# jaeyoungjo99/ELiMaLoc

Hardware: AMD Instinct MI355X
Metric: ICP registrations/sec, 128k-pt scan vs 10M-pt map; pose err vs CPU ref (higher is better)
Workload: dtype f64

## Files before the change

### elimaloc_amd/_lib.py

```python
import ctypes as C
import os

_HERE = os.path.dirname(os.path.abspath(__file__))
LIB_PATH = os.environ.get("ELM_LIB") or os.path.join(_HERE, "libelimaloc_hip.so")

ELM_OK = 0
P2P, GICP, VGICP, AVGICP = 0, 1, 2, 3
MAX_ITER_TRACE = 64
PACKED_SUMS = 32
COMM_ID_BYTES = 128


class ElmError(RuntimeError):
    pass


class RegConfig(C.Structure):
    _fields_ = [
        ("i_max_thread", C.c_int32),
        ("icp_method", C.c_int32),
        ("voxel_search_method", C.c_int32),
        ("use_radar_cov", C.c_int32),
        ("max_iteration", C.c_int32),
        ("b_debug_print", C.c_int32),
# ... 124 lines not shown


class FreeSpaceStatsC(C.Structure):
    _fields_ = [("n_counted", C.c_uint32), ("n_pierced", C.c_uint32), ("n_end_occupied", C.c_uint32), ("n_supported", C.c_uint32),
                ("n_samples", C.c_uint64), ("n_hit_samples", C.c_uint64)]


class RayCastConfigC(C.Structure):
    _fields_ = [("sub", C.c_int32), ("max_steps", C.c_int32), ("min_range_m", C.c_double), ("max_range_m", C.c_double),
                ("cmp_min_range_m", C.c_double), ("cmp_max_range_m", C.c_double), ("tol_m", C.c_double), ("tol_frac", C.c_double),
                ("origin", C.c_double * 3)]


class RayCastStatsC(C.Structure):
    _fields_ = [("n_cast", C.c_uint32), ("n_hit", C.c_uint32), ("n_miss", C.c_uint32), ("n_truncated", C.c_uint32),
                ("n_compared", C.c_uint32), ("n_match", C.c_uint32), ("n_through", C.c_uint32), ("n_front", C.c_uint32),
                ("n_steps", C.c_uint64)]


ALLREDUCE_FN = C.CFUNCTYPE(C.c_int, C.c_void_p, C.c_size_t, C.c_void_p, C.c_void_p)

EXPORTS = [
    "elm_reg_config_default", "elm_ctx_create", "elm_ctx_create_multi", "elm_ctx_group_info", "elm_register_shard", "elm_ctx_destroy", "elm_last_error", "elm_strerror",
    "elm_ctx_synchronize", "elm_ctx_stream", "elm_ctx_set_profiling", "elm_ctx_set_work_counters", "elm_ctx_get_profile", "elm_map_build", "elm_map_destroy", "elm_map_cal_voxel_cov_all",
    "elm_map_cal_point_cov_all", "elm_map_build_neighbourhoods", "elm_map_get_info", "elm_map_empty", "elm_map_download_points",
    "elm_map_download_voxels", "elm_map_find_ground_height", "elm_map_get_correspondences", "elm_align_clouds_local", "elm_scan_upload", "elm_scan_destroy",
    "elm_scan_size", "elm_scan_download", "elm_register", "elm_format_register_log", "elm_register_batch", "elm_register_stream", "elm_register_stream_host", "elm_host_alloc", "elm_host_free", "elm_ctx_measure_h2d", "elm_register_batch_enqueue",
    "elm_register_batch_finish", "elm_deskew", "elm_deskew_downsample", "elm_deskew_prepare", "elm_comm_get_unique_id", "elm_comm_init",
    "elm_comm_destroy", "elm_comm_info", "elm_comm_set_hook", "elm_filter_points_by_distance", "elm_voxel_downsample",
    "elm_get_interpolated_pose", "elm_shape_odom_covariance", "elm_cal_frame_point_cov",
    "elm_ekf_config_default", "elm_ekf_create", "elm_ekf_destroy", "elm_ekf_predict_imu", "elm_ekf_predict", "elm_ekf_update_can", "elm_gps_project", "elm_ekf_update_navsatfix",
    "elm_ekf_update_pose", "elm_ekf_update_pcm_odom", "elm_ekf_get_state", "elm_ekf_publish",
    "elm_ini_load", "elm_ini_destroy", "elm_ini_get_string", "elm_ini_get_int", "elm_ini_get_bool", "elm_ini_get_double",
    "elm_ini_get_array", "elm_pcm_node_config_default", "elm_load_pcm_config", "elm_load_ekf_config", "elm_pcd_load_xyz",
    "elm_free", "elm_scan_from_cloud", "elm_pcm_callback_point_cloud",
    "elm_reloc_config_default", "elm_reloc_make_hypotheses", "elm_map_score_poses", "elm_relocalize",
    "elm_reloc_global_config_default", "elm_map_ground_heights", "elm_reloc_global_hypotheses", "elm_relocalize_global",
    "elm_freespace_config_default", "elm_map_fine_cells", "elm_map_check_free_space",
    "elm_raycast_config_default", "elm_map_raycast",
]


class PcmNodeConfig(C.Structure):
    _fields_ = [("lidar_type", C.c_char * 32), ("lidar_scan_time_end", C.c_int32), ("pcm_voxel_max_point", C.c_int32),
                ("run_deskew", C.c_int32), ("input_index_sampling", C.c_int32), ("lidar_time_delay", C.c_double),
                ("pcm_voxel_size", C.c_double), ("input_max_dist", C.c_double), ("input_voxel_ds_m", C.c_double),
                ("tf_ego_to_lidar", C.c_double * 16)]
# ... 49 lines not shown
                       "(hipcc --offload-arch=gfx950). There is no CPU fallback.")
    L = C.CDLL(LIB_PATH, mode=C.RTLD_GLOBAL)
    vp, dp, fp, ip = C.c_void_p, C.POINTER(C.c_double), C.POINTER(C.c_float), C.POINTER(C.c_int)
    L.elm_reg_config_default.argtypes = [C.POINTER(RegConfig)]
    L.elm_reg_config_default.restype = None
    L.elm_ctx_create.argtypes = [C.c_int, C.POINTER(vp)]
    L.elm_ctx_destroy.argtypes = [vp]
    L.elm_ctx_create_multi.argtypes = [C.POINTER(C.c_int), C.c_int, C.POINTER(vp)]
    L.elm_ctx_group_info.argtypes = [vp, C.POINTER(C.c_int), C.POINTER(C.c_int), C.POINTER(C.c_int), C.c_int]
    L.elm_register_shard.argtypes = [vp, vp, fp, C.c_size_t, C.c_size_t, dp, C.POINTER(RegConfig), C.POINTER(RegResult), C.POINTER(IterTrace), C.c_int]
    L.elm_ctx_destroy.restype = None
    L.elm_last_error.argtypes = [vp]
    L.elm_last_error.restype = C.c_char_p
    L.elm_strerror.argtypes = [C.c_int]
    L.elm_strerror.restype = C.c_char_p
    L.elm_ctx_synchronize.argtypes = [vp]
    L.elm_ctx_stream.argtypes = [vp]
    L.elm_ctx_stream.restype = vp
    L.elm_format_register_log.argtypes = [C.POINTER(RegConfig), C.POINTER(RegResult), C.c_size_t, C.POINTER(IterTrace), C.POINTER(C.c_double),
                                          C.c_double, C.c_char_p, C.c_size_t]
    L.elm_format_register_log.restype = C.c_size_t
    L.elm_ctx_set_profiling.argtypes = [vp, C.c_int]
    L.elm_ctx_set_work_counters.argtypes = [vp, C.c_int]
    L.elm_ctx_get_profile.argtypes = [vp, C.POINTER(Profile), C.c_int]
    L.elm_map_build.argtypes = [vp, fp, C.c_size_t, C.c_double, C.c_int, C.POINTER(vp)]
    L.elm_map_destroy.argtypes = [vp]
    L.elm_map_destroy.restype = None
    L.elm_map_cal_voxel_cov_all.argtypes = [vp]
    L.elm_map_cal_point_cov_all.argtypes = [vp, C.c_double]
    L.elm_map_build_neighbourhoods.argtypes = [vp]
    L.elm_map_get_info.argtypes = [vp, C.POINTER(MapInfo)]
    L.elm_map_empty.argtypes = [vp]
    L.elm_map_download_points.argtypes = [vp, dp, dp, dp, C.c_size_t]
    L.elm_map_download_voxels.argtypes = [vp, C.POINTER(C.c_int32), C.POINTER(C.c_int32), dp, dp, C.c_size_t]
    L.elm_map_find_ground_height.argtypes = [vp, C.c_double, C.c_double, dp, ip]
    L.elm_cal_frame_point_cov.argtypes = [dp, C.c_size_t, C.c_double, C.c_double, C.c_double, dp]
    L.elm_align_clouds_local.argtypes = [vp, C.c_int, dp, dp, dp, dp, C.c_size_t, dp, C.c_double, C.POINTER(RegConfig), dp, dp, dp]
    L.elm_map_get_correspondences.argtypes = [vp, vp, C.c_int, dp, C.c_size_t, C.c_double, C.POINTER(C.c_uint32), C.POINTER(C.c_int32), C.c_size_t, C.POINTER(C.c_size_t)]
    L.elm_scan_upload.argtypes = [vp, fp, C.c_size_t, C.c_size_t, C.POINTER(vp)]
    L.elm_scan_destroy.argtypes = [vp]
    L.elm_scan_destroy.restype = None
    L.elm_scan_size.argtypes = [vp]
    L.elm_scan_size.restype = C.c_size_t
    L.elm_scan_download.argtypes = [vp, fp, C.c_size_t]
    L.elm_deskew_downsample.argtypes = [vp, fp, fp, C.c_size_t, C.POINTER(DeskewTables), C.c_double, C.POINTER(vp), ip]
    L.elm_register.argtypes = [vp, vp, fp, C.c_size_t, dp, C.POINTER(RegConfig), dp, ip, dp, dp,
# ... 96 lines not shown
```

### elimaloc_amd/csrc/elm_api.cpp

```cpp
#include <dlfcn.h>
#include <hip/hip_runtime.h>
#include <math.h>
#include <stdio.h>
#include <stdlib.h>
#include <string.h>
#include <unistd.h>

#include <algorithm>
#include <array>
#include <chrono>
#include <map>
#include <mutex>
#include <new>
#include <set>
#include <string>
#include <thread>
#include <vector>

#include "elm_hostapi.hpp"
#include "elm_internal.hpp"
#include "elm_la.hpp"

using namespace elm;

// ... 48 lines not shown
    g_rccl.comm_init_rank = (nccl_comm_init_rank_t)dlsym(h, "ncclCommInitRank");
    g_rccl.all_reduce = (nccl_all_reduce_t)dlsym(h, "ncclAllReduce");
    g_rccl.comm_destroy = (nccl_comm_destroy_t)dlsym(h, "ncclCommDestroy");
    g_rccl.get_error_string = (nccl_get_error_string_t)dlsym(h, "ncclGetErrorString");
    g_rccl.comm_count = (nccl_comm_query_t)dlsym(h, "ncclCommCount");
    g_rccl.comm_user_rank = (nccl_comm_query_t)dlsym(h, "ncclCommUserRank");
    if (!g_rccl.get_unique_id || !g_rccl.comm_init_rank || !g_rccl.all_reduce || !g_rccl.comm_destroy) {
        if (err) *err = "librccl lacks ncclGetUniqueId/ncclCommInitRank/ncclAllReduce/ncclCommDestroy";
        return false;
    }
    g_rccl.handle = h;
    return true;
}

struct elm_ctx {
    int device = 0;
    uint64_t id = 0;
    hipStream_t stream = nullptr;
    hipStream_t copy_stream = nullptr, order_stream = nullptr, poll_stream = nullptr;
    hipEvent_t ev_iter[4] = {nullptr, nullptr, nullptr, nullptr};
    std::vector<hipEvent_t> ev_groups;
    uint16_t* d_hilbert = nullptr;
    DevBuf d_order_jobs, d_order_tmp, d_arena, d_raw, d_flagged, d_asym;
    DevBuf d_q0, d_q1, d_q2, d_q3, d_q4, d_q5;
    DevBuf d_reloc[16];
    bool work_counters = false;
    void* h_jobs = nullptr;
    size_t h_jobs_cap = 0;
    std::string last_error;
    DevBuf d_scans, d_state, d_partials, d_sums, d_T0, d_trace, d_stage_pts, d_active, d_queue, d_ds;
    int stream_hint_count = 0, stream_hint_slots = 0, stream_hint_iters = 0;
    int* h_active = nullptr;
    int iter_hint = 0;
    int iter_ring[8] = {0, 0, 0, 0, 0, 0, 0, 0};
    unsigned iter_ring_pos = 0;
    const void* iter_key_map = nullptr;
    int iter_key_method = -1, iter_key_batch = 0;
    void* h_state = nullptr;
    size_t h_state_cap = 0;
    void* h_trace = nullptr;
    size_t h_trace_cap = 0;
    void* h_stage = nullptr;
    size_t h_stage_cap = 0;
    std::vector<uint32_t> h_key, h_ord, h_tmp;
    std::vector<struct elm_scan*> scan_free;
    std::vector<std::pair<void*, size_t>> scan_pool;
// ... 161 lines not shown
}

extern "C" void elm_ctx_destroy(elm_ctx* ctx) {
    if (!ctx) return;
    if (ctx->group && !elm_multi::in_worker()) {
        elm_group* g = ctx->group;
        elm_multi::destroy(g);
    }
    {
        std::lock_guard<std::mutex> lk(g_live_mu);
        if (!g_live_ctx.erase(ctx)) return;
    }
    (void)hipSetDevice(ctx->device);
    if (ctx->stream) (void)hipStreamSynchronize(ctx->stream);
    if (ctx->comm && g_rccl.comm_destroy) g_rccl.comm_destroy(ctx->comm);
    for (hipStream_t st : {ctx->copy_stream, ctx->order_stream, ctx->poll_stream})
        if (st) { (void)hipStreamSynchronize(st); (void)hipStreamDestroy(st); }
    for (hipEvent_t e : {ctx->ev_iter[0], ctx->ev_iter[1], ctx->ev_iter[2], ctx->ev_iter[3]})
        if (e) (void)hipEventDestroy(e);
    for (hipEvent_t e : ctx->ev_groups) (void)hipEventDestroy(e);
    if (ctx->d_hilbert) (void)hipFree(ctx->d_hilbert);
    if (ctx->h_jobs) (void)hipHostFree(ctx->h_jobs);
    DevBuf* bufs[] = {&ctx->d_scans, &ctx->d_state, &ctx->d_partials, &ctx->d_sums, &ctx->d_T0, &ctx->d_trace, &ctx->d_stage_pts, &ctx->d_active, &ctx->d_queue, &ctx->d_ds,
                      &ctx->d_order_jobs, &ctx->d_order_tmp, &ctx->d_arena, &ctx->d_raw, &ctx->d_flagged, &ctx->d_asym, &ctx->d_q0, &ctx->d_q1, &ctx->d_q2, &ctx->d_q3, &ctx->d_q4, &ctx->d_q5};
    if (ctx->h_active) (void)hipHostFree(ctx->h_active);
    for (DevBuf* b : bufs)
        if (b->p) (void)hipFree(b->p);
    for (DevBuf& b : ctx->d_reloc)
        if (b.p) (void)hipFree(b.p);
    for (auto& b : ctx->scan_pool) (void)hipFree(b.first);
    for (elm_scan* f : ctx->scan_free) delete f;
    if (ctx->h_state) (void)hipHostFree(ctx->h_state);
    if (ctx->h_trace) (void)hipHostFree(ctx->h_trace);
    if (ctx->h_stage) (void)hipHostFree(ctx->h_stage);
    if (ctx->h_desc) (void)hipHostFree(ctx->h_desc);
    for (hipEvent_t e : ctx->events) (void)hipEventDestroy(e);
    if (ctx->stream) (void)hipStreamDestroy(ctx->stream);
    delete ctx;
}

extern "C" const char* elm_last_error(const elm_ctx* ctx) { return ctx ? ctx->last_error.c_str() : ""; }
extern "C" void* elm_ctx_stream(elm_ctx* ctx) { return ctx ? (void*)ctx->stream : nullptr; }
extern "C" int elm_ctx_set_work_counters(elm_ctx* ctx, int enable) {
    if (!ctx) return ELM_ERR_INVALID;
    if (ctx->in_flight) return ELM_ERR_INVALID;
    if (group_call(ctx)) return elm_multi::set_work_counters(ctx, enable);
    ctx->work_counters = enable != 0;
    return ELM_OK;
}

extern "C" int elm_ctx_set_profiling(elm_ctx* ctx, int enable) {
    if (!ctx) return ELM_ERR_INVALID;
    ctx->profiling = enable != 0;
    return ELM_OK;
}
extern "C" int elm_ctx_get_profile(elm_ctx* ctx, elm_profile* out, int reset) {
    if (!ctx || !out) return ELM_ERR_INVALID;
    *out = ctx->prof;
    if (reset) ctx->prof = elm_profile{};
    return ELM_OK;
}
static int prof_mark(elm_ctx* ctx) {
    if (!ctx->profiling) return ELM_OK;
    if (ctx->events_used == (int)ctx->events.size()) {
        hipEvent_t e;
        HIPCHK(ctx, hipEventCreateWithFlags(&e, hipEventDisableSystemFence));
        ctx->events.push_back(e);
    }
    HIPCHK(ctx, hipEventRecord(ctx->events[ctx->events_used++], ctx->stream));
    return ELM_OK;
// ... 1563 lines not shown
    RegParams rp;
    memset(&rp, 0, sizeof(rp));
    rp.th = cfg->max_search_dist;
    rp.th2 = cfg->max_search_dist * cfg->max_search_dist;
    rp.lm_lambda = cfg->lm_lambda;
    rp.term_thr = cfg->icp_termination_threshold_m;
    rp.min_overlap = cfg->min_overlap_ratio;
    rp.max_fitness = cfg->max_fitness_score;
    rp.method = cfg->icp_method;
    rp.max_iter = cfg->max_iteration;
    rp.uniform_blocks = uniform_blocks;
    rp.radar = pc.radar ? (cfg->use_radar_cov != 0 ? 1 : 2) : 0;
    rp.stats = ctx->work_counters ? 1 : 0;
    rp.radar_var[0] = cfg->range_variance_m;
    rp.radar_var[1] = cfg->azimuth_variance_deg;
    rp.radar_var[2] = cfg->elevation_variance_deg;
    if (pc.asym) {
        int rc;
        if ((rc = dev_reserve(ctx, ctx->d_asym, (size_t)std::max<uint32_t>(blocks, 1) * kAsymRecord * sizeof(double))) != ELM_OK) return rc;
        rp.asym = (double*)ctx->d_asym.p;
        rp.asym_sums = (double*)ctx->d_sums.p + (size_t)n_scans * kSums;
    }
    rp.rank_check = ((ctx->comm || ctx->hook) && !rp.radar && !rp.stats) ? 1 : 0;
    ctx->rp = rp;
    return ELM_OK;
}

static bool reg_args_ok(const elm_ctx* ctx, const elm_map* map, const elm_reg_config* cfg) {
    return map->ctx == ctx && cfg->icp_method >= ELM_P2P && cfg->icp_method <= ELM_AVGICP && !ctx->in_flight;
}

struct StateTail {
    int32_t active;
    int32_t rank_mismatch;
    int32_t _pad0[2];
    uint32_t ds_kept;
    int32_t ds_overflow;
    int32_t _pad1[10];
};
static_assert(sizeof(StateTail) == 64 && offsetof(StateTail, rank_mismatch) == 4 && offsetof(StateTail, ds_kept) == 16 &&
              offsetof(StateTail, ds_overflow) == 20, "the state tail's layout");
static StateTail* state_tail(void* states, int n_scans) { return (StateTail*)((char*)states + (size_t)n_scans * sizeof(ScanState)); }

static size_t trace_bytes(int count) { return (size_t)count * ELM_MAX_ITER_TRACE * sizeof(elm_iter_trace); }
static int reserve_trace(elm_ctx* ctx, int count, elm_iter_trace** d_trace) {
    const size_t tb = trace_bytes(count);
// ... 1169 lines not shown
```

### elimaloc_amd/csrc/elm_internal.hpp

```cpp
#pragma once
#include <hip/hip_runtime.h>
#include <stdint.h>

#include "../../include/elimaloc_hip.h"

namespace elm {

struct __attribute__((aligned(32))) HashSlot {
    int32_t kx, ky, kz;
    int32_t vid;
    uint32_t start;
    uint32_t cnt;
    uint32_t pad0, pad1;
};

struct __attribute__((packed, aligned(4))) Pt3 {
    float x, y, z;
};

struct __attribute__((aligned(16))) GridBlk {
    float x[4], y[4], z[4];
};

struct __attribute__((aligned(64))) VoxRec {
// ... 123 lines not shown
};

struct RegParams {
    double th;
    double th2;
    double lm_lambda;
    double term_thr;
    double min_overlap;
    double max_fitness;
    int32_t method;
    int32_t max_iter;
    uint32_t uniform_blocks;
    int32_t radar;
    int32_t _reserved0;
    int32_t stats;
    uint32_t* flagged;
    int32_t rank_check;
    int32_t _pad_rc;
    double* asym;
    double* asym_sums;
    double radar_var[3];
    const double* query;
    int32_t* q_out;
};
constexpr int kAsymRecord = 16;
constexpr int kRadarRecord = 64;

constexpr int kTileShift = 3, kTile = 1 << kTileShift;
constexpr int kBlock = 256;
constexpr int kInitPack = 8;
struct InitPack {
    ScanDesc d[kInitPack];
    double T0[kInitPack][16];
};
constexpr int kSums = ELM_PACKED_SUMS;

void launch_init_state(hipStream_t s, ScanState* st, const double* T0, int batch, int map_empty, int* active);
void launch_init_pack(hipStream_t s, ScanDesc* scans, ScanState* st, const InitPack& pack, int batch, int map_empty, int* active, const unsigned* n_dev);
void launch_stream_refill(hipStream_t s, ScanDesc* scans, ScanState* st, int slots, const QueueItem* queue, const double* qT0,
                          ScanState* out_state, StreamCtrl* ctrl, int first, int save = 1);
void launch_accumulate_radar(hipStream_t s, const DevMap& m, const ScanDesc* scans, int batch, int total_blocks, ScanState* st, double* partials,
                             const RegParams& rp);
void launch_accumulate_direct(hipStream_t s, const DevMap& m, const ScanDesc* scans, int batch, int total_blocks,
                              ScanState* st, double* partials, const RegParams& rp);
void launch_solve(hipStream_t s, const ScanDesc* scans, int batch, ScanState* st, const double* partials,
                  double* sums, const RegParams& rp, elm_iter_trace* trace, int mode, int* active, const StreamArgs* refill = nullptr);
// ... 129 lines not shown
```

### elimaloc_amd/csrc/elm_k_grid.hip

```cpp
#include <float.h>
#include <algorithm>
#include <hip/hip_runtime.h>

#include "elm_internal.hpp"
#include "elm_la.hpp"
#include "elm_dev_grid.hpp"

namespace elm {

template <int METHOD, int COMPACT, int TILED, int STATS, int WIDE>
__global__ __launch_bounds__(kBlock, (METHOD == ELM_P2P ? (STATS ? 7 : kGridWaves) : kGicpWaves)) void k_accumulate_grid(
       const DevMap m, const ScanDesc* __restrict__ scans, int batch,
                                                                            unsigned total_blocks, const ScanState* __restrict__ st,
                                                                            double* __restrict__ partials, const RegParams rp) {
    constexpr int kStats = (STATS == 1) ? 1 : 0;
    constexpr bool QUERY = STATS == 2;
    constexpr int NV = (METHOD == ELM_P2P) ? (kStats ? kP2PVals : kP2PVals - 3) : kSums;
    __shared__ double s_buf[kRedPass * kBlock];
    __shared__ double s_red[kSums];
    __shared__ int s_res[kBlock];
    __shared__ int s_tst[kStats ? kBlock : 1];
    __shared__ float s_pz[METHOD == ELM_P2P ? kBlock : 1];
    __shared__ unsigned s_st[kStats ? kBlock : 1];
    __shared__ unsigned s_cnt[kBlock / 64];
    const unsigned L = xcd_remap(blockIdx.x, total_blocks);
    const int s = find_scan(scans, batch, L, rp);
    const ScanState& S = st[s];
    if (S.done) return;
    const ScanDesc sd = scans[s];
    if (L >= sd.blk_end) return;
    const unsigned i = (L - sd.blk_begin) * kBlock + threadIdx.x;
    const bool valid = i < sd.n;
    double v[(METHOD == ELM_P2P) ? NV : 1];
#pragma unroll
    for (int k = 0; k < ((METHOD == ELM_P2P) ? NV : 1); ++k) v[k] = 0.0;
    PairSum P;
    if (METHOD != ELM_P2P) pair_sum_zero(P);
    int bj = -1;
    int n_tested = 0;
    float hr2 = __builtin_inff();
    bool hard = false;
    const double h = 0.5 * m.voxel_size;
    const GridBlk* __restrict__ lp = m.grid_blk;
    constexpr unsigned kBlkStep = WIDE ? (unsigned)(sizeof(GridBlk) / 16) : (unsigned)sizeof(GridBlk);
    auto stash_w = [&](double a, double b, double c, double d) {
        double* p = s_buf + threadIdx.x;
        p[4 * kBlock] = a; p[5 * kBlock] = b; p[6 * kBlock] = c; p[7 * kBlock] = d;
    };
    auto load_g = [&](double& gx, double& gy, double& gz, float& pxf, float& pyf) {
        const double* p = s_buf + threadIdx.x;
        gx = p[4 * kBlock]; gy = p[5 * kBlock]; gz = p[6 * kBlock];
        const double w = p[7 * kBlock];
        pxf = __int_as_float(__double2loint(w)); pyf = __int_as_float(__double2hiint(w));
    };
    auto transform = [&](const float4 pf, double& px, double& py, double& pz, double& gx, double& gy, double& gz) {
        px = pf.x; py = pf.y; pz = pf.z;
        gx = ((S.T[0] * px + S.T[4] * py) + S.T[8] * pz) + S.T[12];
        gy = ((S.T[1] * px + S.T[5] * py) + S.T[9] * pz) + S.T[13];
        gz = ((S.T[2] * px + S.T[6] * py) + S.T[10] * pz) + S.T[14];
    };
    if (valid) {
        double px, py, pz, gx, gy, gz;
        float4 pf = make_float4(0.f, 0.f, 0.f, 0.f);
        if (QUERY) {
            gx = rp.query[3 * (size_t)i]; gy = rp.query[3 * (size_t)i + 1]; gz = rp.query[3 * (size_t)i + 2];
            px = py = pz = 0.0;
        } else {
            const Pt3 p3 = sd.pts[i];
            pf = make_float4(p3.x, p3.y, p3.z, 0.f);
            transform(pf, px, py, pz, gx, gy, gz);
        }
        const GridAxis ax = grid_axis(gx, m), ay = grid_axis(gy, m), az = grid_axis(gz, m);
        unsigned stat = 0;
        if (kStats && !TILED) {
            const int ux = ax.f - m.vx0, uy = ay.f - m.vy0, uz = az.f - m.vz0;
            const bool in_box = (unsigned)ux < (unsigned)m.vnx && (unsigned)uy < (unsigned)m.vny && (unsigned)uz < (unsigned)m.vnz;
            const unsigned sidx = in_box ? ((unsigned)ux * (unsigned)m.vny + (unsigned)uy) * (unsigned)m.vnz + (unsigned)uz : 0u;
            stat = m.vox_stat[sidx];
            stat = in_box ? stat : 0u;
        }
        float rho_u = 3e38f;
        int bx0, bx1, by0, by1, bz0, bz1;
        int ox, oy, oz;
        float dxo, dyo, dzo;
        grid_lean(ax, bx0, bx1, rho_u, ox, dxo);
        grid_lean(ay, by0, by1, rho_u, oy, dyo);
        grid_lean(az, bz0, bz1, rho_u, oz, dzo);
        (void)oz; (void)dzo;
        const int rx0 = bx0 - m.gx0, rx1 = bx1 - m.gx0, ry0 = by0 - m.gy0, ry1 = by1 - m.gy0, rz0 = bz0 - m.gz0, rz1 = bz1 - m.gz0;
        const bool inside = rx0 >= 0 && rx1 < m.gnx && rx0 <= rx1 && ry0 >= 0 && ry1 < m.gny && ry0 <= ry1 && rz0 >= 0 && rz1 < m.gnz && rz0 <= rz1;
        unsigned sb[4];
        int cb[5];
        cb[0] = 0;
        const float ex_ = fmaxf(dxo * (float)h - 1e-6f, 0.f), ey_ = fmaxf(dyo * (float)h - 1e-6f, 0.f);
        const float Bx = fminf(ex_ * ex_, 1e36f), By = fminf(ey_ * ey_, 1e36f);
        const bool xfirst = Bx <= By, has_x = rx1 != rx0, has_y = ry1 != ry0;
        unsigned s0[4], s1[4], s2[4];
        bool ok[4];
        ok[0] = inside;
        ok[1] = inside && (xfirst ? has_x : has_y);
        ok[2] = inside && (xfirst ? has_y : has_x);
        ok[3] = inside && has_x && has_y;
        if (!TILED) {
            const int own_x = ox ? rx1 : rx0, own_y = oy ? ry1 : ry0;
            const unsigned base = ((unsigned)own_x * (unsigned)m.gny + (unsigned)own_y) * (unsigned)m.gnz + (unsigned)rz0;
            const unsigned xs = (unsigned)m.gny * (unsigned)m.gnz, ys = (unsigned)m.gnz;
            const unsigned cx_n = ox ? base - xs : base + xs, cy_n = oy ? base - ys : base + ys, cd = ox ? cy_n - xs : cy_n + xs;
            unsigned cellv[4];
            cellv[0] = base; cellv[1] = xfirst ? cx_n : cy_n; cellv[2] = xfirst ? cy_n : cx_n; cellv[3] = cd;
#pragma unroll
            for (int k = 0; k < 4; ++k) {
                const uint32_t* e = m.grid_start + (ok[k] ? cellv[k] : 0u);
// ... 1 lines not shown
            }
        } else {
            const int own_x = ox ? rx1 : rx0, oth_x = ox ? rx0 : rx1, own_y = oy ? ry1 : ry0, oth_y = oy ? ry0 : ry1;
            int cxv[4], cyv[4];
            cxv[0] = own_x; cyv[0] = own_y;
            cxv[1] = xfirst ? oth_x : own_x; cyv[1] = xfirst ? own_y : oth_y;
            cxv[2] = xfirst ? own_x : oth_x; cyv[2] = xfirst ? oth_y : own_y;
            cxv[3] = oth_x; cyv[3] = oth_y;
#pragma unroll
            for (int k = 0; k < 4; ++k) {
                int zc0, nzc;
                const uint32_t* e = col_cells<1>(m, ok[k] ? cxv[k] : 0, ok[k] ? cyv[k] : 0, rz0, rz1, zc0, nzc);
                s0[k] = e[0]; s1[k] = e[nzc]; s2[k] = s1[k];
            }
        }
        float rr = (rho_u < 1e30f) ? (rho_u * (float)h - 1.1e-6f) * 0.999998f : 1e18f;
        float rr2 = (rr > 0.f) ? rr * rr * 0.999999f : -1.f;
        float ghx = (float)gx, ghy = (float)gy, ghz = (float)gz;
        const float eg = (fabsf(ghx) + fabsf(ghy) + fabsf(ghz)) * 5.9604652e-08f;
        float egrr = (2.0f * eg * fmaxf(rr, 0.f) + eg * eg) * 1.000001f;
        float egblk = (7.0f * eg * (float)h + eg * eg) * 1.000001f;
        float L1 = fminf(Bx, By), L2 = fmaxf(Bx, By), L3 = (Bx + By) * 0.999999f;
        asm volatile("" : "+v"(rr2), "+v"(ghx), "+v"(ghy), "+v"(ghz), "+v"(egrr), "+v"(egblk), "+v"(L1), "+v"(L2), "+v"(L3));
        stash_w(gx, gy, gz, __hiloint2double(__float_as_int(pf.y), __float_as_int(pf.x)));
        if (METHOD == ELM_P2P) s_pz[threadIdx.x] = pf.z;
        if (kStats) s_st[threadIdx.x] = stat;
        {
            int b0v[4], b1v[4];
#pragma unroll
            for (int k = 0; k < 4; ++k) {
                b0v[k] = ok[k] ? (int)s0[k] : 0;
                b1v[k] = ok[k] ? (int)((rz1 > rz0 || TILED) ? s2[k] : s1[k]) : 0;
            }
#pragma unroll
            for (int k = 0; k < 4; ++k) {
                sb[k] = (unsigned)(b0v[k] - cb[k]) * kBlkStep;
                cb[k + 1] = cb[k] + (b1v[k] - b0v[k]);
            }
        }
        {
            int nblk = cb[4];
            const f32x2 gxy = {ghx, ghy}, gzz = {ghz, 0.f};
            unsigned m1 = 0x7F800000u, m2 = 0x7F800000u;
            unsigned jb = 0;
            for (int t0 = 0; t0 < nblk; t0 += kBlocksPerTrip) {
                unsigned pb[kBlocksPerTrip];
#pragma unroll
                for (int w = 0; w < kBlocksPerTrip; ++w) {
// ... 5 lines not shown
                }
                GridBlk B[kBlocksPerTrip];
#pragma unroll
                for (int w = 0; w < kBlocksPerTrip; ++w)
                    B[w] = *reinterpret_cast<const GridBlk*>(reinterpret_cast<const char*>(lp) + (WIDE ? ((size_t)pb[w] << 4) : (size_t)pb[w]));
                __builtin_amdgcn_sched_barrier(0);
#pragma unroll
                for (int w = 0; w < kBlocksPerTrip; ++w) {
                    f32x2 da, db;
                    blk_dist_h(B[w], gxy, gzz, da, db);
                    const unsigned was = m1;
                    two_smallest(da.x, 0u, m1, m2);
                    two_smallest(da.y, 1u, m1, m2);
                    two_smallest(db.x, 2u, m1, m2);
                    two_smallest(db.y, 3u, m1, m2);
                    jb = (m1 != was) ? pb[w] : jb;
                }
                const float dbest = __uint_as_float(m1 & ~3u);
                const float best = (dbest < rr2) ? (dbest + dbest * 7.62939453125e-06f + 2.0f * egrr) * 1.000001f : __builtin_inff();
                nblk = (L1 > best) ? cb[1] : ((L2 > best) ? cb[2] : ((L3 > best) ? cb[3] : nblk));
            }
            n_tested = 4 * nblk;
            hard = true;
            if (jb > 0) {
                const float d1 = __uint_as_float(m1 & ~3u), d2 = __uint_as_float(m2 & ~3u);
                const float r2 = d1 + d1 * 3.814697265625e-06f + egrr;
                hr2 = d1 + d1 * 3.814697265625e-06f + egblk;
                if (d2 - d2 * 3.814697265625e-06f > r2 + egrr && r2 < rr2) {
                    bj = (int)(jb / kBlkStep) * 4 + (int)(m1 & 3u);
                    hard = false;
                }
            }
        }
    }
    const unsigned long long hm = __ballot(hard);
    const unsigned lane = threadIdx.x & 63u, wave = threadIdx.x >> 6;
    if (lane == 0) s_cnt[wave] = (unsigned)__popcll(hm);
    __syncthreads();
    unsigned n_hard = 0, my_slot = 0;
#pragma unroll
    for (unsigned w = 0; w < kBlock / 64; ++w) {
        my_slot += (w < wave) ? s_cnt[w] : 0u;
        n_hard += s_cnt[w];
    }
    my_slot += (unsigned)__popcll(hm & ((1ull << lane) - 1ull));
    if (n_hard) {
        GridHardRec* __restrict__ s_rec = reinterpret_cast<GridHardRec*>(s_buf);
        if (hard) {
            GridHardRec r;
            float pxf_, pyf_;
            load_g(r.gx, r.gy, r.gz, pxf_, pyf_);
            r.r2 = hr2; r._pad = 0.f;
            s_rec[my_slot] = r;
        }
        __syncthreads();
        constexpr unsigned LPI = kHardLanes;
        const unsigned rl = threadIdx.x & (LPI - 1u), row = threadIdx.x / LPI;
        for (unsigned it0 = 0; it0 < n_hard; it0 += kBlock / LPI) {
            const unsigned it = it0 + row;
            if (it0 + (threadIdx.x & ~63u) / LPI >= n_hard) break;
            const bool live = it < n_hard;
            const GridHardRec R = s_rec[live ? it : 0];
            int win, walked;
            grid_ball_walk<TILED, LPI>(m, lp, R, live, rl, lane, win, walked);
            if (kStats) walked = group_sum_int<LPI>(walked);
            if (rl == 0 && live) {
                s_res[it] = win;
                if (kStats) s_tst[it] = walked;
            }
        }
        __syncthreads();
        if (hard) {
            bj = s_res[my_slot];
            if (kStats) n_tested += s_tst[my_slot];
        }
        __syncthreads();
    }
    if (QUERY) {
        if (valid) {
            double gx, gy, gz;
            float pxf, pyf;
            load_g(gx, gy, gz, pxf, pyf);
            int out = -2;
            if (bj >= 0) {
                const Pt3 q = blk_point(lp, bj);
                const double ex = (double)q.x - gx, ey = (double)q.y - gy, ez = (double)q.z - gz;
                if ((ex * ex + ey * ey) + ez * ez < rp.th2) out = (int)m.grid_idx[bj];
            } else if ((gx * gx + gy * gy) + gz * gz < rp.th2) {
                out = -1;
            }
            rp.q_out[i] = out;
        }
        return;
    }
    if (valid) {
        double gx, gy, gz;
        float pxf, pyf;
        load_g(gx, gy, gz, pxf, pyf);
        const double px = pxf, py = pyf, pz = (METHOD == ELM_P2P) ? (double)s_pz[threadIdx.x] : 0.0;
        const unsigned stat = kStats ? s_st[threadIdx.x] : 0u;
        float bx = 0.f, by = 0.f, bz = 0.f;
        int bidx = -1;
        const bool range_known = METHOD != ELM_P2P && !hard && bj >= 0 && (12.25 * h * h) * 1.0001 < rp.th2;
        if (bj >= 0) {
            if (!range_known) {
                const Pt3 q = blk_point(lp, bj);
                bx = q.x; by = q.y; bz = q.z;
            }
            bidx = bj;
        }
        const double ex = (double)bx - gx, ey = (double)by - gy, ez = (double)bz - gz;
        const double bd2 = range_known ? 0.0 : (ex * ex + ey * ey) + ez * ez;
        const double c_cand = (double)(stat & 0xFFFFu);
        const double c_occ = (double)(stat >> 16);
        const double c_tested = (double)n_tested + (hard ? kFallbackUnit : 0.0);
        if (METHOD == ELM_P2P) {
            if (bd2 < rp.th2) pair_p2p(v, S.Rinv, px, py, pz, ex, ey, ez, bd2, rp);
            if (kStats) { v[NV - 3] = c_cand; v[NV - 2] = c_occ; v[NV - 1] = c_tested; }
        } else {
            const double dfin = (bidx >= 0) ? bd2 : (gx * gx + gy * gy) + gz * gz;
            if (COMPACT == 2) {
// ... 97 lines not shown
```

### elimaloc_amd/registration.py

```python
import ctypes as C
import enum

import numpy as np

from . import _lib
from ._lib import (ElmError, FreeSpaceConfigC, FreeSpaceStatsC, RayCastConfigC, RayCastStatsC, GlobalRelocConfigC, GlobalRelocStats, RegConfig, RegResult, IterTrace, MapInfo, RelocCandidate, RelocConfigC,
                   check)


class IcpMethod(enum.IntEnum):
    P2P = 0
    GICP = 1
    VGICP = 2
    AVGICP = 3


def RegistrationConfig(**kw):
    cfg = RegConfig()
    _lib.lib().elm_reg_config_default(C.byref(cfg))
    for k, v in kw.items():
        if not hasattr(cfg, k):
            raise AttributeError(f"RegistrationConfig has no field {k}")
        setattr(cfg, k, int(v) if k in ("icp_method", "max_iteration", "i_max_thread", "use_radar_cov") else v)
    return cfg
# ... 123 lines not shown
        check(_lib.lib().elm_ctx_group_info(self._h, C.byref(n), C.byref(ex), ids, 64), self._h, "elm_ctx_group_info")
        return n.value, ex.value, [ids[i] for i in range(n.value)]

    def close(self):
        if getattr(self, "_h", None):
            _lib.lib().elm_ctx_destroy(self._h)
            self._h = None

    def __del__(self):
        try:
            self.close()
        except Exception:
            pass

    def synchronize(self):
        check(_lib.lib().elm_ctx_synchronize(self._h), self._h, "elm_ctx_synchronize")

    @property
    def stream(self):
        return _lib.lib().elm_ctx_stream(self._h)

    def set_work_counters(self, on=True):
        check(_lib.lib().elm_ctx_set_work_counters(self._h, int(bool(on))), self._h, "elm_ctx_set_work_counters")

    def set_profiling(self, on=True):
        check(_lib.lib().elm_ctx_set_profiling(self._h, int(bool(on))), self._h, "elm_ctx_set_profiling")

    def get_profile(self, reset=False):
        p = _lib.Profile()
        check(_lib.lib().elm_ctx_get_profile(self._h, C.byref(p), int(bool(reset))), self._h, "elm_ctx_get_profile")
        return dict(accumulate_launches=int(p.accumulate_launches), solve_steps=int(p.solve_steps),
                    accumulate_ms=float(p.accumulate_ms), solve_ms=float(p.solve_ms))

    def measure_h2d(self, host_ptr, nbytes, reps=5):
        g = C.c_double(0.0)
        check(_lib.lib().elm_ctx_measure_h2d(self._h, C.c_void_p(host_ptr), int(nbytes), int(reps), C.byref(g)), self._h, "elm_ctx_measure_h2d")
        return g.value

    @staticmethod
    def comm_unique_id():
        buf = (C.c_char * _lib.COMM_ID_BYTES)()
        check(_lib.lib().elm_comm_get_unique_id(C.cast(buf, C.c_void_p)), None, "elm_comm_get_unique_id")
        return bytes(buf)

    def comm_init(self, rank, nranks, id_bytes):
        buf = (C.c_char * _lib.COMM_ID_BYTES).from_buffer_copy(id_bytes)
# ... 613 lines not shown
```

### include/elimaloc_hip.h

```cpp
#ifndef ELIMALOC_HIP_H
#define ELIMALOC_HIP_H

#include <stddef.h>
#include <stdint.h>

#ifdef __cplusplus
extern "C" {
#endif

#define ELM_OK 0
#define ELM_ERR_INVALID -1
#define ELM_ERR_DEVICE -2
#define ELM_ERR_NO_DEVICE -3
#define ELM_ERR_COMM -4
#define ELM_ERR_UNSUPPORTED -5
#define ELM_ERR_IO -6
#define ELM_ERR_ALLOC -7

#define ELM_MAX_ITER_TRACE 64

typedef struct elm_ctx elm_ctx;
typedef struct elm_map elm_map;
typedef struct elm_scan elm_scan;

// ... 72 lines not shown
    uint64_t nbr_entries;
    uint64_t index_bytes;
    uint64_t index_part_bytes[4];
    uint64_t n_list_voxels;
} elm_map_info;


int elm_ctx_create(int device_id, elm_ctx** out);
void elm_ctx_destroy(elm_ctx* ctx);
const char* elm_last_error(const elm_ctx* ctx);
const char* elm_strerror(int status);
int elm_ctx_synchronize(elm_ctx* ctx);
void* elm_ctx_stream(elm_ctx* ctx);

typedef struct elm_profile {
    uint64_t accumulate_launches;
    uint64_t solve_steps;
    double accumulate_ms;
    double solve_ms;
} elm_profile;
int elm_ctx_set_profiling(elm_ctx* ctx, int enable);
int elm_ctx_set_work_counters(elm_ctx* ctx, int enable);
int elm_ctx_get_profile(elm_ctx* ctx, elm_profile* out, int reset);

int elm_map_build(elm_ctx* ctx, const float* xyz, size_t n, double voxel_size, int max_points_per_voxel,
                  elm_map** out);
void elm_map_destroy(elm_map* map);
int elm_map_cal_voxel_cov_all(elm_map* map);
int elm_map_cal_point_cov_all(elm_map* map, double d_search_dist);
int elm_map_build_neighbourhoods(elm_map* map);
int elm_map_get_info(const elm_map* map, elm_map_info* info);
int elm_map_empty(const elm_map* map);
int elm_map_download_points(const elm_map* map, double* xyz, double* cov9, double* mean3, size_t cap);
int elm_map_download_voxels(const elm_map* map, int32_t* key3, int32_t* npts, double* cov9, double* mean3,
                            size_t cap);
int elm_map_get_correspondences(elm_ctx* ctx, const elm_map* map, int what, const double* xyz, size_t n, double max_dist,
                                uint32_t* src_index, int32_t* tgt_index, size_t cap, size_t* n_pairs);

int elm_align_clouds_local(elm_ctx* ctx, int method, const double* src_local, const double* tgt_xyz, const double* tgt_cov9,
                           const double* src_cov9, size_t n, const double last_icp_pose[16], double trans_th,
                           const elm_reg_config* cfg, double T_out[16], double local_cov[36], double* fitness_score);

int elm_map_find_ground_height(const elm_map* map, double x, double y, double* ground_z, int* found);

int elm_scan_upload(elm_ctx* ctx, const float* xyz, size_t n, size_t n_total, elm_scan** out);
void elm_scan_destroy(elm_scan* scan);
// ... 246 lines not shown
```

Before: 98170.

## Reuse previous-iteration nearest neighbour when the point stays inside a safe radius

For P2P grid registration, each point's transformed position, its matched map index and a conservative safety radius (based on the gap to the second-best candidate and the distance to the voxel face) are stored after each iteration. From the third iteration on, points that moved less than that radius keep their previous match. Only the remaining points are compacted into a per-block queue and searched. This cuts the grid nearest-neighbour search work as ICP converges, at the cost of extra global writes and reads per point, shared-memory compaction and extra synchronisation. Optional counters are added to report how many points reuse their match.

```diff
diff --git a/elimaloc_amd/_lib.py b/elimaloc_amd/_lib.py
--- a/elimaloc_amd/_lib.py
+++ b/elimaloc_amd/_lib.py
@@ -170,7 +170,7 @@
 
 EXPORTS = [
     "elm_reg_config_default", "elm_ctx_create", "elm_ctx_create_multi", "elm_ctx_group_info", "elm_register_shard", "elm_ctx_destroy", "elm_last_error", "elm_strerror",
-    "elm_ctx_synchronize", "elm_ctx_stream", "elm_ctx_set_profiling", "elm_ctx_set_work_counters", "elm_ctx_get_profile", "elm_map_build", "elm_map_destroy", "elm_map_cal_voxel_cov_all",
+    "elm_ctx_synchronize", "elm_ctx_stream", "elm_ctx_set_profiling", "elm_ctx_set_work_counters", "elm_ctx_set_carry_counters", "elm_ctx_get_carry_counters", "elm_ctx_get_profile", "elm_map_build", "elm_map_destroy", "elm_map_cal_voxel_cov_all",
     "elm_map_cal_point_cov_all", "elm_map_build_neighbourhoods", "elm_map_get_info", "elm_map_empty", "elm_map_download_points",
     "elm_map_download_voxels", "elm_map_find_ground_height", "elm_map_get_correspondences", "elm_align_clouds_local", "elm_scan_upload", "elm_scan_destroy",
     "elm_scan_size", "elm_scan_download", "elm_register", "elm_format_register_log", "elm_register_batch", "elm_register_stream", "elm_register_stream_host", "elm_host_alloc", "elm_host_free", "elm_ctx_measure_h2d", "elm_register_batch_enqueue",
@@ -266,6 +266,8 @@
     L.elm_format_register_log.restype = C.c_size_t
     L.elm_ctx_set_profiling.argtypes = [vp, C.c_int]
     L.elm_ctx_set_work_counters.argtypes = [vp, C.c_int]
+    L.elm_ctx_set_carry_counters.argtypes = [vp, C.c_int]
+    L.elm_ctx_get_carry_counters.argtypes = [vp, C.POINTER(C.c_double), C.POINTER(C.c_double)]
     L.elm_ctx_get_profile.argtypes = [vp, C.POINTER(Profile), C.c_int]
     L.elm_map_build.argtypes = [vp, fp, C.c_size_t, C.c_double, C.c_int, C.POINTER(vp)]
     L.elm_map_destroy.argtypes = [vp]
diff --git a/elimaloc_amd/csrc/elm_api.cpp b/elimaloc_amd/csrc/elm_api.cpp
--- a/elimaloc_amd/csrc/elm_api.cpp
+++ b/elimaloc_amd/csrc/elm_api.cpp
@@ -94,6 +94,8 @@
     std::vector<hipEvent_t> ev_groups;
     uint16_t* d_hilbert = nullptr;
     DevBuf d_order_jobs, d_order_tmp, d_arena, d_raw, d_flagged, d_asym;
+    DevBuf d_carry_g, d_carry_bj, d_carry_cnt;
+    bool carry_failed = false;
     DevBuf d_q0, d_q1, d_q2, d_q3, d_q4, d_q5;
     DevBuf d_reloc[16];
     bool work_counters = false;
@@ -301,7 +303,7 @@
     if (ctx->d_hilbert) (void)hipFree(ctx->d_hilbert);
     if (ctx->h_jobs) (void)hipHostFree(ctx->h_jobs);
     DevBuf* bufs[] = {&ctx->d_scans, &ctx->d_state, &ctx->d_partials, &ctx->d_sums, &ctx->d_T0, &ctx->d_trace, &ctx->d_stage_pts, &ctx->d_active, &ctx->d_queue, &ctx->d_ds,
-                      &ctx->d_order_jobs, &ctx->d_order_tmp, &ctx->d_arena, &ctx->d_raw, &ctx->d_flagged, &ctx->d_asym, &ctx->d_q0, &ctx->d_q1, &ctx->d_q2, &ctx->d_q3, &ctx->d_q4, &ctx->d_q5};
+                      &ctx->d_order_jobs, &ctx->d_order_tmp, &ctx->d_arena, &ctx->d_raw, &ctx->d_flagged, &ctx->d_asym, &ctx->d_carry_g, &ctx->d_carry_bj, &ctx->d_carry_cnt, &ctx->d_q0, &ctx->d_q1, &ctx->d_q2, &ctx->d_q3, &ctx->d_q4, &ctx->d_q5};
     if (ctx->h_active) (void)hipHostFree(ctx->h_active);
     for (DevBuf* b : bufs)
         if (b->p) (void)hipFree(b->p);
@@ -325,6 +327,33 @@
     if (ctx->in_flight) return ELM_ERR_INVALID;
     if (group_call(ctx)) return elm_multi::set_work_counters(ctx, enable);
     ctx->work_counters = enable != 0;
+    return ELM_OK;
+}
+
+extern "C" int elm_ctx_set_carry_counters(elm_ctx* ctx, int enable) {
+    if (!ctx || ctx->in_flight || group_call(ctx)) return ELM_ERR_INVALID;
+    HIPCHK(ctx, hipSetDevice(ctx->device));
+    HIPCHK(ctx, hipStreamSynchronize(ctx->stream));
+    if (!enable) {
+        if (ctx->d_carry_cnt.p) HIPCHK(ctx, hipFree(ctx->d_carry_cnt.p));
+        ctx->d_carry_cnt = DevBuf{};
+        return ELM_OK;
+    }
+    int rc;
+    if ((rc = dev_reserve(ctx, ctx->d_carry_cnt, 2 * sizeof(unsigned long long))) != ELM_OK) return rc;
+    HIPCHK(ctx, hipMemset(ctx->d_carry_cnt.p, 0, 2 * sizeof(unsigned long long)));
+    return ELM_OK;
+}
+extern "C" int elm_ctx_get_carry_counters(elm_ctx* ctx, double* tested_points, double* reused_points) {
+    if (!ctx || ctx->in_flight || !tested_points || !reused_points) return ELM_ERR_INVALID;
+    unsigned long long h[2] = {0, 0};
+    if (ctx->d_carry_cnt.p) {
+        HIPCHK(ctx, hipSetDevice(ctx->device));
+        HIPCHK(ctx, hipStreamSynchronize(ctx->stream));
+        HIPCHK(ctx, hipMemcpy(h, ctx->d_carry_cnt.p, sizeof(h), hipMemcpyDeviceToHost));
+    }
+    *tested_points = (double)h[0];
+    *reused_points = (double)h[1];
     return ELM_OK;
 }
 
@@ -1934,6 +1963,20 @@
         rp.asym_sums = (double*)ctx->d_sums.p + (size_t)n_scans * kSums;
     }
     rp.rank_check = ((ctx->comm || ctx->hook) && !rp.radar && !rp.stats) ? 1 : 0;
+    constexpr uint64_t kCarryMaxBytes = 2ull << 30;
+    if (pc.use_grid && !pc.radar && cfg->icp_method == ELM_P2P && !rp.stats && cfg->max_iteration > 2 && blocks > 0 && !ctx->carry_failed &&
+        (uint64_t)blocks * kBlock * 20ull <= kCarryMaxBytes && !check_mode("no_carry")) {
+        const size_t n_rec = (size_t)blocks * kBlock;
+        if (dev_reserve(ctx, ctx->d_carry_g, n_rec * sizeof(float4)) == ELM_OK && dev_reserve(ctx, ctx->d_carry_bj, n_rec * sizeof(uint32_t)) == ELM_OK) {
+            rp.carry_g = (float4*)ctx->d_carry_g.p;
+            rp.carry_bj = (uint32_t*)ctx->d_carry_bj.p;
+            rp.carry_cnt = (unsigned long long*)ctx->d_carry_cnt.p;
+        } else {
+            (void)hipGetLastError();
+            ctx->carry_failed = true;
+            ctx->last_error.clear();
+        }
+    }
     ctx->rp = rp;
     return ELM_OK;
 }
diff --git a/elimaloc_amd/csrc/elm_internal.hpp b/elimaloc_amd/csrc/elm_internal.hpp
--- a/elimaloc_amd/csrc/elm_internal.hpp
+++ b/elimaloc_amd/csrc/elm_internal.hpp
@@ -169,6 +169,9 @@
     double radar_var[3];
     const double* query;
     int32_t* q_out;
+    float4* carry_g;
+    uint32_t* carry_bj;
+    unsigned long long* carry_cnt;
 };
 constexpr int kAsymRecord = 16;
 constexpr int kRadarRecord = 64;
diff --git a/elimaloc_amd/csrc/elm_k_grid.hip b/elimaloc_amd/csrc/elm_k_grid.hip
--- a/elimaloc_amd/csrc/elm_k_grid.hip
+++ b/elimaloc_amd/csrc/elm_k_grid.hip
@@ -16,6 +16,7 @@
     constexpr int kStats = (STATS == 1) ? 1 : 0;
     constexpr bool QUERY = STATS == 2;
     constexpr int NV = (METHOD == ELM_P2P) ? (kStats ? kP2PVals : kP2PVals - 3) : kSums;
+    constexpr bool CARRY = METHOD == ELM_P2P && STATS == 0;
     __shared__ double s_buf[kRedPass * kBlock];
     __shared__ double s_red[kSums];
     __shared__ int s_res[kBlock];
@@ -23,6 +24,8 @@
     __shared__ float s_pz[METHOD == ELM_P2P ? kBlock : 1];
     __shared__ unsigned s_st[kStats ? kBlock : 1];
     __shared__ unsigned s_cnt[kBlock / 64];
+    __shared__ int s_own[CARRY ? kBlock : 1];
+    __shared__ unsigned char s_q[CARRY ? kBlock : 1];
     const unsigned L = xcd_remap(blockIdx.x, total_blocks);
     const int s = find_scan(scans, batch, L, rp);
     const ScanState& S = st[s];
@@ -47,8 +50,8 @@
         double* p = s_buf + threadIdx.x;
         p[4 * kBlock] = a; p[5 * kBlock] = b; p[6 * kBlock] = c; p[7 * kBlock] = d;
     };
-    auto load_g = [&](double& gx, double& gy, double& gz, float& pxf, float& pyf) {
-        const double* p = s_buf + threadIdx.x;
+    auto load_g = [&](unsigned slot, double& gx, double& gy, double& gz, float& pxf, float& pyf) {
+        const double* p = s_buf + slot;
         gx = p[4 * kBlock]; gy = p[5 * kBlock]; gz = p[6 * kBlock];
         const double w = p[7 * kBlock];
         pxf = __int_as_float(__double2loint(w)); pyf = __int_as_float(__double2hiint(w));
@@ -59,11 +62,55 @@
         gy = ((S.T[1] * px + S.T[5] * py) + S.T[9] * pz) + S.T[13];
         gz = ((S.T[2] * px + S.T[6] * py) + S.T[10] * pz) + S.T[14];
     };
-    if (valid) {
+    const int cmode = (CARRY && rp.carry_g != nullptr) ? min(S.iters, 2) : 0;
+    const bool rd = CARRY && cmode == 2;
+    const size_t crec = (size_t)L * kBlock;
+    unsigned n_search = kBlock;
+    auto owner = [&]() -> unsigned { return rd ? (unsigned)s_q[threadIdx.x] : threadIdx.x; };
+    if (rd) {
+        bool need = false;
+        if (valid) {
+            const Pt3 p3 = sd.pts[i];
+            const float4 cg4 = rp.carry_g[crec + threadIdx.x];
+            const int cbj = (int)rp.carry_bj[crec + threadIdx.x];
+            double px, py, pz, gx, gy, gz;
+            transform(make_float4(p3.x, p3.y, p3.z, 0.f), px, py, pz, gx, gy, gz);
+            stash_w(gx, gy, gz, __hiloint2double(__float_as_int(p3.y), __float_as_int(p3.x)));
+            s_pz[threadIdx.x] = p3.z;
+            const double dx = gx - (double)cg4.x, dy = gy - (double)cg4.y, dz = gz - (double)cg4.z;
+            const double bq = (double)cg4.w;
+            need = !(cg4.w > 0.f && (dx * dx + dy * dy) + dz * dz < bq * bq);
+            if (!need) s_own[threadIdx.x] = cbj;
+        }
+        const unsigned long long nm = __ballot(need);
+        const unsigned lane_ = threadIdx.x & 63u, wave_ = threadIdx.x >> 6;
+        if (lane_ == 0) s_cnt[wave_] = (unsigned)__popcll(nm);
+        __syncthreads();
+        unsigned n_need = 0, q_slot = 0;
+#pragma unroll
+        for (unsigned w = 0; w < kBlock / 64; ++w) {
+            q_slot += (w < wave_) ? s_cnt[w] : 0u;
+            n_need += s_cnt[w];
+        }
+        q_slot += (unsigned)__popcll(nm & ((1ull << lane_) - 1ull));
+        if (need) s_q[q_slot] = (unsigned char)threadIdx.x;
+        __syncthreads();
+        n_search = n_need;
+        if (rp.carry_cnt != nullptr && threadIdx.x == 0) {
+            const unsigned n_wg = min((unsigned)kBlock, sd.n - (L - sd.blk_begin) * kBlock);
+            atomicAdd(rp.carry_cnt, (unsigned long long)n_wg);
+            atomicAdd(rp.carry_cnt + 1, (unsigned long long)(n_wg - n_need));
+        }
+    }
+    if (valid && threadIdx.x < n_search) {
         double px, py, pz, gx, gy, gz;
         float4 pf = make_float4(0.f, 0.f, 0.f, 0.f);
         if (QUERY) {
             gx = rp.query[3 * (size_t)i]; gy = rp.query[3 * (size_t)i + 1]; gz = rp.query[3 * (size_t)i + 2];
+            px = py = pz = 0.0;
+        } else if (rd) {
+            float pxf_, pyf_;
+            load_g(owner(), gx, gy, gz, pxf_, pyf_);
             px = py = pz = 0.0;
         } else {
             const Pt3 p3 = sd.pts[i];
@@ -88,6 +135,11 @@
         grid_lean(az, bz0, bz1, rho_u, oz, dzo);
         (void)oz; (void)dzo;
         const int rx0 = bx0 - m.gx0, rx1 = bx1 - m.gx0, ry0 = by0 - m.gy0, ry1 = by1 - m.gy0, rz0 = bz0 - m.gz0, rz1 = bz1 - m.gz0;
+        if (CARRY && cmode) {
+            const float ux = (float)(ax.cg & 1) + ax.fr, uy = (float)(ay.cg & 1) + ay.fr, uz = (float)(az.cg & 1) + az.fr;
+            const float fu = fminf(fminf(fminf(ux, 2.f - ux), fminf(uy, 2.f - uy)), fminf(uz, 2.f - uz));
+            s_res[threadIdx.x] = __float_as_int((bx1 != bx0 && by1 != by0 && bz1 != bz0) ? fu * (float)h : 0.f);
+        }
         const bool inside = rx0 >= 0 && rx1 < m.gnx && rx0 <= rx1 && ry0 >= 0 && ry1 < m.gny && ry0 <= ry1 && rz0 >= 0 && rz1 < m.gnz && rz0 <= rz1;
         unsigned sb[4];
         int cb[5];
@@ -135,8 +187,10 @@
         float egblk = (7.0f * eg * (float)h + eg * eg) * 1.000001f;
         float L1 = fminf(Bx, By), L2 = fmaxf(Bx, By), L3 = (Bx + By) * 0.999999f;
         asm volatile("" : "+v"(rr2), "+v"(ghx), "+v"(ghy), "+v"(ghz), "+v"(egrr), "+v"(egblk), "+v"(L1), "+v"(L2), "+v"(L3));
-        stash_w(gx, gy, gz, __hiloint2double(__float_as_int(pf.y), __float_as_int(pf.x)));
-        if (METHOD == ELM_P2P) s_pz[threadIdx.x] = pf.z;
+        if (!rd) {
+            stash_w(gx, gy, gz, __hiloint2double(__float_as_int(pf.y), __float_as_int(pf.x)));
+            if (METHOD == ELM_P2P) s_pz[threadIdx.x] = pf.z;
+        }
         if (kStats) s_st[threadIdx.x] = stat;
         {
             int b0v[4], b1v[4];
@@ -188,6 +242,7 @@
             }
             n_tested = 4 * nblk;
             hard = true;
+            float beta = 0.f;
             if (jb > 0) {
                 const float d1 = __uint_as_float(m1 & ~3u), d2 = __uint_as_float(m2 & ~3u);
                 const float r2 = d1 + d1 * 3.814697265625e-06f + egrr;
@@ -195,7 +250,22 @@
                 if (d2 - d2 * 3.814697265625e-06f > r2 + egrr && r2 < rr2) {
                     bj = (int)(jb / kBlkStep) * 4 + (int)(m1 & 3u);
                     hard = false;
+                    if (CARRY && cmode) {
+                        const int cb4 = cb[4];
+                        float lsk = __builtin_inff();
+                        if (nblk < cb4) lsk = fminf((nblk <= cb[1]) ? L1 : ((nblk <= cb[2]) ? L2 : L3), L3);
+                        const float lo2 = fminf(fminf(d2 - d2 * 3.814697265625e-06f - egrr, lsk), rr2);
+                        const float gap = (__builtin_sqrtf(fmaxf(lo2, 0.f)) - __builtin_sqrtf(r2)) * 0.5f;
+                        const float face = __int_as_float(s_res[threadIdx.x]);
+                        const float eg_ = (fabsf(gxy.x) + fabsf(gxy.y) + fabsf(gzz.x)) * 5.9604652e-08f;
+                        beta = fminf(gap, face) * 0.99999f - 1e-6f - eg_;
+                    }
                 }
+            }
+            if (CARRY && cmode) {
+                const size_t ri = crec + owner();
+                rp.carry_g[ri] = make_float4(gxy.x, gxy.y, gzz.x, beta);
+                rp.carry_bj[ri] = (uint32_t)bj;
             }
         }
     }
@@ -215,7 +285,7 @@
         if (hard) {
             GridHardRec r;
             float pxf_, pyf_;
-            load_g(r.gx, r.gy, r.gz, pxf_, pyf_);
+            load_g(owner(), r.gx, r.gy, r.gz, pxf_, pyf_);
             r.r2 = hr2; r._pad = 0.f;
             s_rec[my_slot] = r;
         }
@@ -242,11 +312,16 @@
         }
         __syncthreads();
     }
+    if (rd) {
+        if (threadIdx.x < n_search) s_own[s_q[threadIdx.x]] = bj;
+        __syncthreads();
+        bj = valid ? s_own[threadIdx.x] : -1;
+    }
     if (QUERY) {
         if (valid) {
             double gx, gy, gz;
             float pxf, pyf;
-            load_g(gx, gy, gz, pxf, pyf);
+            load_g(threadIdx.x, gx, gy, gz, pxf, pyf);
             int out = -2;
             if (bj >= 0) {
                 const Pt3 q = blk_point(lp, bj);
@@ -262,7 +337,7 @@
     if (valid) {
         double gx, gy, gz;
         float pxf, pyf;
-        load_g(gx, gy, gz, pxf, pyf);
+        load_g(threadIdx.x, gx, gy, gz, pxf, pyf);
         const double px = pxf, py = pyf, pz = (METHOD == ELM_P2P) ? (double)s_pz[threadIdx.x] : 0.0;
         const unsigned stat = kStats ? s_st[threadIdx.x] : 0u;
         float bx = 0.f, by = 0.f, bz = 0.f;
diff --git a/elimaloc_amd/registration.py b/elimaloc_amd/registration.py
--- a/elimaloc_amd/registration.py
+++ b/elimaloc_amd/registration.py
@@ -169,6 +169,14 @@
 
     def set_work_counters(self, on=True):
         check(_lib.lib().elm_ctx_set_work_counters(self._h, int(bool(on))), self._h, "elm_ctx_set_work_counters")
+
+    def set_carry_counters(self, on=True):
+        check(_lib.lib().elm_ctx_set_carry_counters(self._h, int(bool(on))), self._h, "elm_ctx_set_carry_counters")
+
+    def get_carry_counters(self):
+        a, b = C.c_double(0.0), C.c_double(0.0)
+        check(_lib.lib().elm_ctx_get_carry_counters(self._h, C.byref(a), C.byref(b)), self._h, "elm_ctx_get_carry_counters")
+        return a.value, b.value
 
     def set_profiling(self, on=True):
         check(_lib.lib().elm_ctx_set_profiling(self._h, int(bool(on))), self._h, "elm_ctx_set_profiling")
diff --git a/include/elimaloc_hip.h b/include/elimaloc_hip.h
--- a/include/elimaloc_hip.h
+++ b/include/elimaloc_hip.h
@@ -118,6 +118,8 @@
 int elm_ctx_set_profiling(elm_ctx* ctx, int enable);
 int elm_ctx_set_work_counters(elm_ctx* ctx, int enable);
 int elm_ctx_get_profile(elm_ctx* ctx, elm_profile* out, int reset);
+int elm_ctx_set_carry_counters(elm_ctx* ctx, int enable);
+int elm_ctx_get_carry_counters(elm_ctx* ctx, double* tested_points, double* reused_points);
 
 int elm_map_build(elm_ctx* ctx, const float* xyz, size_t n, double voxel_size, int max_points_per_voxel,
                   elm_map** out);
```

New measurement: 90730. -7.6%, worse.
